# tuanir/fantoch

Hardware: AMD Instinct MI355X
Metric: region configs evaluated/sec (1/2/4/8 GPUs), synthetic 64-region planet n=7 f=1,2 (higher is better)
Workload: dtype u32

## Files before the change

### fantoch_amd/csrc/bote_group.hip

```cpp
#include "bote_fast.hpp"
#include "bote_launch.hpp"

#define AS3 __attribute__((address_space(3)))

namespace bote {

constexpr int GROUP_MAX_BD = 1024;
#ifndef BOTE_GROUP_WAVES
#define BOTE_GROUP_WAVES 5
#endif
#ifndef BOTE_GROUP_WAVES_PERM
#define BOTE_GROUP_WAVES_PERM 4
#endif

__host__ __device__ constexpr int cmax(int a, int b) { return a > b ? a : b; }
template <bool B>
struct BoolC {
  static constexpr bool value = B;
};

template <int N>
struct GCfg {
  using QC = QCfg<N>;
  static constexpr int F = N - 3;
  static constexpr int FP = (F + 1) / 2;
  static constexpr int KQ = cmax(cmax(QC::qa1, QC::maxf >= 2 ? QC::qa2 : 0), cmax(QC::qe, 3)) - 1;
  static_assert(KQ <= N - 1, "quorum larger than the config");
  static constexpr bool PERM = N <= 7 && QC::NL == 2;
  static constexpr bool RX = N <= 7;
  static_assert(!RX || (F <= 4 && KQ <= 4), "position table holds 4 fixed members");
};

__host__ __device__ inline uint32_t gline_rx_bytes(const FastArgs& a, int N) { return N <= 7 && a.grx ? a.ns * 16 : 0u; }
__host__ __device__ inline uint32_t gline_bytes(const FastArgs& a, int N, int KQ) {
  const int F = N - 3, FP = (F + 1) / 2;
  return (gline_rx_bytes(a, N) + a.cq_stride * 8 + (uint32_t)(FP * KQ + 2 * F) * 4 + 15) & ~15u;
}

__host__ __device__ inline uint32_t lines_wave_bytes(const FastArgs& a) {
  return (a.gslots * (a.cq_stride * 8 + 4) + 15) & ~15u;
}

struct GroupLds {
  size_t lines_or_qtab;
  size_t cqt;
  size_t rqt;
  size_t srv;
  size_t lrec;
  size_t cs2;
  size_t vcol;
  size_t vcol32;
  size_t glines;
  size_t top;
  size_t cand;
  size_t tmp;
  size_t thr;
  size_t lock;
  size_t bins;
  size_t digest;
  size_t total;
};

enum : int {
  LOCK_MERGE = 0,
  LOCK_SCORE = 1,
  LOCK_COV = 2,
};

__host__ __device__ inline GroupLds group_layout(const FastArgs& a, int N, int NLW, int KQ, bool perm) {
  const auto a16 = [](size_t o) { return (o + 15) & ~(size_t)15; };
  GroupLds l;
  size_t o = 0;
  l.lines_or_qtab = o; o += perm ? (size_t)(a.gbd / 64) * lines_wave_bytes(a) : ((size_t)N * NLW) << a.gqsh;
  o = a16(o);
  l.cqt = o; o += (size_t)a.R * a.cq_stride * 8;
  l.rqt = o; o += a.rq_separate ? (size_t)a.R * a.rq_stride * 8 : 0;
  l.srv = o; o += (size_t)a.ns * 4;
  o = (o + 7) & ~(size_t)7;
  l.lrec = o; o += (size_t)a.ns * 8;
  o = a16(o);
  l.cs2 = o; o += (size_t)a.ns * 8;
  l.vcol = o; o += (size_t)a.ns * 8;
  l.vcol32 = o; o += (size_t)a.ns * 4;
  o = a16(o);
  l.glines = o; o += (size_t)(a.gbd / 64) * gline_bytes(a, N, KQ);
  o = a16(o);
  l.top = o; o += (size_t)a.n_obj * a.K * 16;
  l.cand = o; o += (size_t)64 * 16;
  l.tmp = o; o += (size_t)a.K * 16;
  l.thr = o; o += (size_t)MAXOBJ * 16;
  l.lock = o; o += 48;
  o = a16(o);
  l.bins = o; o += perm && (a.keys || a.gbins) ? (size_t)(a.gbd / 64) * N * 256 : 0;
  o = a16(o);
  l.digest = o; o += (size_t)a.gbd * 8;
  l.total = o;
  return l;
}

template <int N>
static size_t group_smem_n(const FastArgs& a) {
  return group_layout(a, N, QCfg<N>::NL <= 2 ? 1 : 2, GCfg<N>::KQ, GCfg<N>::PERM).total;
}

bool group_uses_lines(uint32_t n) {
  switch (n) {
#define PL_CASE(NN) case NN: return GCfg<NN>::PERM;
    PL_CASE(4) PL_CASE(5) PL_CASE(6) PL_CASE(7)
#undef PL_CASE
    default: return false;
  }
}

size_t group_smem_bytes(const FastArgs& a, uint32_t n) {
  switch (n) {
#define SM_CASE(NN) case NN: return group_smem_n<NN>(a);
    SM_CASE(4) SM_CASE(5) SM_CASE(6) SM_CASE(7) SM_CASE(8) SM_CASE(9) SM_CASE(10) SM_CASE(11) SM_CASE(12)
    SM_CASE(13) SM_CASE(14) SM_CASE(15) SM_CASE(16)
#undef SM_CASE
    default: return 0;
  }
}

__device__ __forceinline__ uint32_t uni(uint32_t x) { return __builtin_amdgcn_readfirstlane(x); }

__device__ __forceinline__ uint64_t uni64(uint64_t x) {
  return ((uint64_t)uni((uint32_t)(x >> 32)) << 32) | uni((uint32_t)x);
}

__device__ __forceinline__ uint32_t lds_base(const void* p) { return (uint32_t)(uintptr_t)(const AS3 void*)p; }
__device__ __forceinline__ uint32_t l16(uint32_t a) { return *(const AS3 uint16_t*)(uintptr_t)a; }
__device__ __forceinline__ uint32_t l32(uint32_t a) { return *(const AS3 uint32_t*)(uintptr_t)a; }
__device__ __forceinline__ uint2 l64(uint32_t a) {
  const uint64_t v = *(const AS3 uint64_t*)(uintptr_t)a;
  return make_uint2((uint32_t)v, (uint32_t)(v >> 32));
}
typedef uint32_t u32x4 __attribute__((ext_vector_type(4)));
__device__ __forceinline__ uint4 l128(uint32_t a) {
  const u32x4 v = *(const AS3 u32x4*)(uintptr_t)a;
  return make_uint4(v.x, v.y, v.z, v.w);
}
__device__ __forceinline__ float lf32(uint32_t a) { return *(const AS3 float*)(uintptr_t)a; }
__device__ __forceinline__ void s16(uint32_t a, uint32_t v) { *(AS3 uint16_t*)(uintptr_t)a = (uint16_t)v; }
__device__ __forceinline__ void s32(uint32_t a, uint32_t v) { *(AS3 uint32_t*)(uintptr_t)a = v; }
__device__ __forceinline__ void s64(uint32_t a, uint32_t lo, uint32_t hi) {
  *(AS3 uint64_t*)(uintptr_t)a = (uint64_t)lo | ((uint64_t)hi << 32);
}
__device__ __forceinline__ void s128(uint32_t a, uint4 v) {
  u32x4 w;
  w.x = v.x;
  w.y = v.y;
  w.z = v.z;
  w.w = v.w;
  *(AS3 u32x4*)(uintptr_t)a = w;
}

__device__ __forceinline__ void wave_sync() {
  __builtin_amdgcn_fence(__ATOMIC_RELEASE, "workgroup");
  __builtin_amdgcn_wave_barrier();
  __builtin_amdgcn_fence(__ATOMIC_ACQUIRE, "workgroup");
}

__device__ __forceinline__ us2 ld_pair(uint32_t a, uint32_t b) {
  us2 r;
  r.x = *(const AS3 unsigned short*)(uintptr_t)a;
  r.y = *(const AS3 unsigned short*)(uintptr_t)b;
  return r;
}

__device__ __forceinline__ us2 pk_min(us2 a, us2 b) { return __builtin_elementwise_min(a, b); }
__device__ __forceinline__ us2 pk_max(us2 a, us2 b) { return __builtin_elementwise_max(a, b); }

template <int P>
__device__ __forceinline__ void sort_network_pk(uint32_t* a) {
#pragma unroll
  for (int p = 1; p < P; p <<= 1) {
#pragma unroll
    for (int k = p; k >= 1; k >>= 1) {
#pragma unroll
      for (int j = k % p; j + k < P; j += 2 * k) {
#pragma unroll
        for (int i = 0; i < k; ++i) {
          if (i + j + k < P && (i + j) / (2 * p) == (i + j + k) / (2 * p)) {
            const us2 x = as_us2(a[i + j]), y = as_us2(a[i + j + k]);
            a[i + j] = as_u32(pk_min(x, y));
            a[i + j + k] = as_u32(pk_max(x, y));
          }
        }
      }
    }
  }
}

template <int KA, int KY, int KO, class T>
__device__ __forceinline__ void merge_lists(const T* A, const T* y, T* L) {
#pragma unroll
  for (int k = 0; k < KO; ++k) {
    T z = k < KA ? A[k < KA ? k : 0] : y[0];
    bool have = k < KA;
#pragma unroll
    for (int j = 1; j <= KY && j <= k + 1; ++j) {
      const int i = k + 1 - j;
      if (i > KA) continue;
      const T c = i == 0 ? y[j - 1] : __builtin_elementwise_max(A[i > 0 ? i - 1 : 0], y[j - 1]);
      z = have ? __builtin_elementwise_min(z, c) : c;
      have = true;
    }
    L[k] = z;
  }
}

__device__ __forceinline__ int32_t score_tlo(uint64_t tkey, uint32_t nc) {
  if (tkey == ~0ull) return INT32_MIN;
  const uint64_t ob = ~tkey;
  const uint64_t bits = (ob >> 63) ? (ob & 0x7FFFFFFFFFFFFFFFull) : ~ob;
  const double tscore = __longlong_as_double((long long)bits);
  if (!(tscore == tscore)) return INT32_MIN;
  const double b = (tscore - 1e-6) * (double)nc;
  if (b <= -2147483648.0) return INT32_MIN;
  if (b > 1073741824.0) return 1073741824;
  return (int32_t)ceil(b);
}

__device__ __forceinline__ float cov_tf32(uint64_t tkey) {
  if (tkey == ~0ull) return __builtin_inff();
  return (float)__longlong_as_double((long long)tkey) * (1.0f + 0x1p-10f);
}

template <int KA, int KY, class T>
__device__ __forceinline__ void merge_top4(const T* A, const T* y, T* L) {
  static_assert(KA >= 1 && KY >= 1 && KA + KY >= 4 && KA <= 4 && KY <= 4, "4 smallest of KA + KY >= 4 entries");
  T B[4];
#pragma unroll
  for (int i = 0; i < 4; ++i) {
    const int j = 3 - i;
    if (i < KA && j < KY) B[i] = __builtin_elementwise_min(A[i < KA ? i : 0], y[j < KY ? j : 0]);
    else if (i < KA) B[i] = A[i < KA ? i : 0];
    else B[i] = y[j < KY ? j : 0];
  }
  auto ce = [&](int a, int b) {
    const T lo = __builtin_elementwise_min(B[a], B[b]);
    B[b] = __builtin_elementwise_max(B[a], B[b]);
    B[a] = lo;
  };
  ce(0, 2);
  ce(1, 3);
  ce(0, 1);
  ce(2, 3);
#pragma unroll
  for (int i = 0; i < 4; ++i) L[i] = B[i];
}

template <int KA, int KY, int KO, class T>
__device__ __forceinline__ void merge_k(const T* A, const T* y, T* L) {
  if constexpr (KO == 4 && KA + KY >= 4) merge_top4<KA, KY>(A, y, L);
  else merge_lists<KA, KY, KO>(A, y, L);
}

__device__ __forceinline__ void wave_topk(const TopkLds& t, int* lock, uint32_t nc, int n_obj, uint32_t K,
                                          const uint64_t (&key)[MAXOBJ], const bool (&ok)[MAXOBJ], uint64_t rank) {
  const uint32_t lane = threadIdx.x & 63;
  const int KL = (int)K;
  if (lane == 0) {
    while (atomicCAS(lock + LOCK_MERGE, 0, 1) != 0) __builtin_amdgcn_s_sleep(2);
  }
  __builtin_amdgcn_wave_barrier();
  __builtin_amdgcn_fence(__ATOMIC_ACQUIRE, "workgroup");
  const uint32_t rlo = (uint32_t)rank, rhi = (uint32_t)(rank >> 32);
#pragma unroll
  for (int o = 0; o < MAXOBJ; ++o) {
    if (o >= n_obj) break;
    Rec* top = t.top + o * KL;
    const Rec mine = Rec{key[o], rank};
    const bool p = ok[o] && rec_lt(mine, t.thr[o]);
    const uint64_t m = __ballot(p);
    if (m == 0) continue;
    const bool h0 = (int)lane < KL, h1 = (int)lane + 64 < KL;
    const Rec x0 = h0 ? top[lane] : rec_max(), x1 = h1 ? top[lane + 64] : rec_max();
    int r0 = (int)lane, r1 = (int)lane + 64;
    int rc = p ? lower_bound_rec(top, KL, mine) : 0;
    const uint32_t klo = (uint32_t)key[o], khi = (uint32_t)(key[o] >> 32);
    for (uint64_t mm = m; mm; mm &= mm - 1) {
      const int src = __builtin_ctzll(mm);
      const uint64_t ck = ((uint64_t)(uint32_t)__builtin_amdgcn_readlane(khi, src) << 32) |
                          (uint32_t)__builtin_amdgcn_readlane(klo, src);
      const uint64_t cr = ((uint64_t)(uint32_t)__builtin_amdgcn_readlane(rhi, src) << 32) |
                          (uint32_t)__builtin_amdgcn_readlane(rlo, src);
      const Rec c = Rec{ck, cr};
      r0 += rec_lt(c, x0);
      r1 += rec_lt(c, x1);
      rc += rec_lt(c, mine);
    }
    if (h0 && r0 < KL) t.tmp[r0] = x0;
    if (h1 && r1 < KL) t.tmp[r1] = x1;
    if (p && rc < KL) t.tmp[rc] = mine;
    wave_sync();
#pragma unroll
    for (int h = 0; h < KP / 64; ++h)
      if ((int)lane + 64 * h < KL) top[lane + 64 * h] = t.tmp[lane + 64 * h];
    wave_sync();
    if (lane == 0 && rec_lt(top[K - 1], t.thr[o])) {
      t.thr[o] = top[K - 1];
      if (o == 0) lock[LOCK_SCORE] = score_tlo(top[K - 1].key, nc);
      if (o == 3) lock[LOCK_COV] = __float_as_int(cov_tf32(top[K - 1].key));
    }
    wave_sync();
  }
  __builtin_amdgcn_fence(__ATOMIC_RELEASE, "workgroup");
  if (lane == 0) atomicExch(lock + LOCK_MERGE, 0);
}

template <class FX, class FY>
__device__ __forceinline__ int cov2_sign(float Vx, uint32_t Sx, float Vy, uint32_t Sy, const FX& dVx, const FY& dVy) {
  const float fx = (float)Sx, fy = (float)Sy;
  const float x = Vx * (fy * fy), y = Vy * (fx * fx);
  const float d = x - y, tol = 0x1p-18f * fmaxf(x, y);
  if (d < -tol) return -1;
  if (d > tol) return 1;
  const double sx = (double)Sx, sy = (double)Sy;
  const double X = dVx() * (sy * sy), Y = dVy() * (sx * sx);
  const double D = X - Y, T = 0x1p-32 * fmax(X, Y);
  return D < -T ? -1 : (D > T ? 1 : 0);
}

template <class FX, class FY>
__device__ __forceinline__ int cov2_sign_ge(float Vx, uint32_t Sx, float Vy, uint32_t Sy, float fy2, const FX& dVx,
                                            const FY& dVy) {
  const float fx = (float)Sx;
  const float x = Vx * fy2, y = Vy * (fx * fx);
  constexpr float c = 1.0f - 0x1p-18f;
  if (x * c >= y) return 1;
  if (x < y * c) return -1;
  const double sx = (double)Sx, sy = (double)Sy;
  const double X = dVx() * (sy * sy), Y = dVy() * (sx * sx);
  const double D = X - Y, T = 0x1p-32 * fmax(X, Y);
  return D < -T ? -1 : (D > T ? 1 : 0);
}

__device__ __forceinline__ float u64_to_f32(uint64_t x) {
  return __builtin_fmaf((float)(uint32_t)(x >> 32), 0x1p32f, (float)(uint32_t)x);
}

struct GroupCtx {
  bool sid;
  bool use_rx;
  uint32_t LB;
  uint32_t qtab;
  uint32_t cqt, rqt;
  uint32_t thra;
  uint32_t cstride, rstride;
  uint32_t nc, nq, rem;
  uint32_t lines, keys;
  uint32_t rxt;
  uint32_t mfl;
  uint32_t upk;
  uint32_t fS1;
  uint32_t fVf;
};

template <bool LINES>
__device__ __forceinline__ void nearest_quad(const GroupCtx& cx, uint32_t ll, uint32_t c0, uint32_t c1, uint32_t c2,
                                             uint32_t g8, us2& lo, us2& hi) {
  const us2 J1 = {1, 1}, J2 = {2, 2};
  const uint2 wa = l64(c0 + g8);
  if constexpr (LINES) {
    const uint2 wl = l64(ll + g8);
    lo = pk_min(as_us2(wa.x), as_us2(wl.x));
    hi = pk_min(as_us2(wa.y), as_us2(wl.y));
  } else {
    const uint2 wb = l64(c1 + g8), wc = l64(c2 + g8), wf = l64(cx.mfl + g8);
    lo = pk_min(pk_min(as_us2(wa.x), as_us2(wb.x) | J1), pk_min(as_us2(wc.x) | J2, as_us2(wf.x)));
    hi = pk_min(pk_min(as_us2(wa.y), as_us2(wb.y) | J1), pk_min(as_us2(wc.y) | J2, as_us2(wf.y)));
  }
}

template <bool LINES>
__device__ __forceinline__ void nearest_quad_pair(const GroupCtx& cx, uint32_t ll, uint32_t c0, uint32_t c1, uint32_t c2,
                                                  uint32_t g16, us2& lo0, us2& hi0, us2& lo1, us2& hi1) {
  const us2 J1 = {1, 1}, J2 = {2, 2};
  const uint4 wa = l128(c0 + g16);
  if constexpr (LINES) {
    const uint4 wl = l128(ll + g16);
    lo0 = pk_min(as_us2(wa.x), as_us2(wl.x));
    hi0 = pk_min(as_us2(wa.y), as_us2(wl.y));
    lo1 = pk_min(as_us2(wa.z), as_us2(wl.z));
    hi1 = pk_min(as_us2(wa.w), as_us2(wl.w));
  } else {
    const uint4 wb = l128(c1 + g16), wc = l128(c2 + g16), wf = l128(cx.mfl + g16);
    lo0 = pk_min(pk_min(as_us2(wa.x), as_us2(wb.x) | J1), pk_min(as_us2(wc.x) | J2, as_us2(wf.x)));
    hi0 = pk_min(pk_min(as_us2(wa.y), as_us2(wb.y) | J1), pk_min(as_us2(wc.y) | J2, as_us2(wf.y)));
    lo1 = pk_min(pk_min(as_us2(wa.z), as_us2(wb.z) | J1), pk_min(as_us2(wc.z) | J2, as_us2(wf.z)));
    hi1 = pk_min(pk_min(as_us2(wa.w), as_us2(wb.w) | J1), pk_min(as_us2(wc.w) | J2, as_us2(wf.w)));
  }
}

constexpr uint32_t GROUP_UNROLL = 4;
#ifndef BOTE_BIN_FIRST
#define BOTE_BIN_FIRST 0
#endif
#ifndef BOTE_BIN_FIRST_XK
#define BOTE_BIN_FIRST_XK 1
#endif
constexpr uint32_t BIN_UB = 4;
template <int N, bool DEF, bool SI, bool RXC, bool XK, bool BN = false>
__global__ void __launch_bounds__(XK ? GROUP_XK_MAX_BD : GROUP_MAX_BD,
                                  XK ? BOTE_GROUP_WAVES_XK : (GCfg<N>::PERM ? BOTE_GROUP_WAVES_PERM : BOTE_GROUP_WAVES))
    sweep_group_kernel(FastArgs a) {
  GroupCtx cx;
  cx.sid = SI || a.srv_identity;
  constexpr bool S32 = SI;
  cx.use_rx = GCfg<N>::RX && (SI ? RXC : a.grx != 0);
  using QC = QCfg<N>;
  using GC = GCfg<N>;
  constexpr int NL = QC::NL;
  constexpr int NLW = NL <= 2 ? 1 : 2;
  constexpr int F = GC::F;
  constexpr int FP = GC::FP;
  constexpr int KQ = GC::KQ;
  constexpr int PV = Pow2<N - 1>::v;
  constexpr int PF = Pow2<F>::v;
  constexpr bool PERM = GC::PERM;
  constexpr bool BIN = XK || (PERM && BN);
  constexpr bool BIN_FIRST = BIN && (XK ? BOTE_BIN_FIRST_XK : BOTE_BIN_FIRST);
  static_assert(!XK || (PERM && DEF), "the extended key set runs on the PERM kernels with the default objectives");
  using QT = QTab<N, XK>;
  constexpr int NT = QT::NT;
  extern __shared__ __align__(16) unsigned char smem[];
  const GroupLds off = group_layout(a, N, NLW, KQ, PERM);
  cx.LB = lds_base(smem);
  cx.qtab = cx.LB + (uint32_t)off.lines_or_qtab;
  cx.cqt = cx.LB + (uint32_t)off.cqt;
  cx.rqt = cx.LB + (uint32_t)(a.rq_separate ? off.rqt : off.cqt);
  uint32_t* srv = (uint32_t*)(smem + off.srv);
  uint2* lrec = (uint2*)(smem + off.lrec);
  uint64_t* cs2 = (uint64_t*)(smem + off.cs2);
  double* vcol = (double*)(smem + off.vcol);
  float* vcol32 = (float*)(smem + off.vcol32);
  const uint64_t* binom = a.binom;
  TopkLds tk;
  tk.top = (Rec*)(smem + off.top);
  tk.cand = (Rec*)(smem + off.cand);
  tk.tmp = (Rec*)(smem + off.tmp);
  tk.thr = (Rec*)(smem + off.thr);
  cx.thra = cx.LB + (uint32_t)off.thr;
  tk.cnt = nullptr;
  int* lock = (int*)(smem + off.lock);
  const uint32_t tid = threadIdx.x, lane = tid & 63, wid = tid >> 6, BD = blockDim.x, WPB = BD >> 6;
  const uint32_t qsh = a.gqsh;

  {
    const uint32_t cw = a.R * a.cq_stride * 2;
    const uint32_t* src = (const uint32_t*)a.cqt;
    uint32_t* dst = (uint32_t*)(smem + off.cqt);
    for (uint32_t i = tid; i < cw; i += BD) dst[i] = src[i];
    if (a.rq_separate) {
      const uint32_t rw = a.R * a.rq_stride * 2;
      const uint32_t* rs = (const uint32_t*)a.rqt;
      uint32_t* rd = (uint32_t*)(smem + off.rqt);
      for (uint32_t i = tid; i < rw; i += BD) rd[i] = rs[i];
    }
  }
  for (uint32_t i = tid; i < a.ns; i += BD) srv[i] = a.srv[i];
  for (uint32_t i = tid; i < (uint32_t)a.n_obj * a.K; i += BD) tk.top[i] = rec_max();
  if (tid < MAXOBJ) tk.thr[tid] = a.tseed && tid < a.n_obj ? Rec{a.tseed[tid], ~0ull} : rec_max();
  if (tid == 0) {
    lock[LOCK_MERGE] = 0;
    lock[LOCK_SCORE] = score_tlo(a.tseed && a.n_obj ? a.tseed[0] : ~0ull, a.nc);
    lock[LOCK_COV] = __float_as_int(cov_tf32(a.tseed && a.n_obj > 3 ? a.tseed[3] : ~0ull));
  }
  if (a.smin && a.smin_wave && lane < a.n_obj)
    a.smin[(size_t)lane * gridDim.x * WPB + (size_t)blockIdx.x * WPB + wid] = ~0ull;
  if constexpr (BIN)
    for (uint32_t i = tid; i < (BD >> 6) * N * 64; i += BD) ((uint32_t*)(smem + off.bins))[i] = 0;
  ((uint64_t*)(smem + off.digest))[tid] = 0;
  __syncthreads();
  cx.cstride = a.cq_stride * 8;
  cx.rstride = a.rq_stride * 8;
  for (uint32_t i = tid; i < a.ns; i += BD) {
    const uint32_t col = cx.cqt + srv[i] * cx.cstride;
    uint64_t c1 = 0, c2 = 0;
    for (uint32_t c = 0; c < a.nc; ++c) {
      uint64_t v = l16(col + 2 * c) >> LAT_SHIFT;
      c1 += v;
      c2 += v * v;
    }
    cs2[i] = c2;
    const double v = (double)((uint64_t)a.nc * c2 - c1 * c1);
    vcol[i] = v;
    vcol32[i] = (float)v;
    const float w = v > 0.0 ? (float)(1.0 / sqrt(v)) : __builtin_inff();
    lrec[i] = make_uint2((uint32_t)c1, __float_as_uint(w));
  }
  __syncthreads();

  cx.nc = a.nc;
  cx.nq = cx.nc >> 2;
  cx.rem = cx.nc & 3;
  const uint32_t qlane = cx.qtab + tid * 4;
  cx.lines = cx.qtab + wid * lines_wave_bytes(a);
  cx.keys = cx.lines + a.gslots * cx.cstride;
  const uint32_t gl = cx.LB + (uint32_t)off.glines + wid * gline_bytes(a, N, KQ);
  cx.rxt = gl;
  cx.mfl = gl + gline_rx_bytes(a, N);
  cx.upk = cx.mfl + cx.cstride;
  cx.fS1 = cx.upk + FP * KQ * 4;
  cx.fVf = cx.fS1 + F * 4;
  const double pnc1 = a.p_fmean * (double)cx.nc, pnc2 = a.p_emean * (double)cx.nc;
  uint64_t valid_cnt = 0;
  const uint32_t dofs =
      uni(cx.LB + (uint32_t)off.digest + wid * 512u - 2u * (cx.LB + (uint32_t)off.bins + wid * (N * 256u)));
  auto digest_add = [&](uint32_t binb_, uint64_t d) {
    uint32_t ad;
    asm("v_lshl_add_u32 %0, %1, 1, %2" : "=v"(ad) : "v"(binb_), "s"(dofs));
    __hip_atomic_fetch_add((AS3 uint64_t*)(uintptr_t)ad, d, __ATOMIC_RELAXED, __HIP_MEMORY_SCOPE_WAVEFRONT);
  };

  bool static_done = false;
  const uint32_t wsh = a.wshards ? a.wshards : 1u, wx = blockIdx.x % wsh;
  unsigned int* const tctr = a.wctr + 32 * wx;
  uint32_t cnext = 0;
  if (a.nwchunks && lane == 0) cnext = atomicAdd(tctr, 1u);
  for (;;) {
  uint64_t r, rend;
  uint32_t chunk = ~0u;
  if (a.nwchunks) {
    const uint32_t c = wx + wsh * uni(cnext);
    if (c >= a.nwchunks) break;
    if (lane == 0) cnext = atomicAdd(tctr, 1u);
    chunk = c;
    PSTAT(a, 13, true);
    r = uni64(a.wchunks[c]);
    rend = a.smin ? min(r + 64ull * a.ssteps, a.re) : uni64(a.wchunks[c + 1]);
    GASSERT(a, a.rb <= r && r <= rend && rend <= a.re, 0);
  } else {
    if (static_done) break;
    static_done = true;
    const uint64_t nwaves = (uint64_t)gridDim.x * WPB;
    const uint64_t gw = (uint64_t)blockIdx.x * WPB + wid;
    const uint64_t total = a.re - a.rb;
    r = uni64(a.rb + (uint64_t)(((unsigned __int128)total * gw) / nwaves));
    rend = uni64(a.rb + (uint64_t)(((unsigned __int128)total * (gw + 1)) / nwaves));
  }

  if (r < rend) {
    uint32_t hq[F];
    uint64_t base = 0;
    if (a.wstate && chunk != ~0u) {
      const uint64_t* st = a.wstate + 4 * (size_t)chunk;
      base = uni64(st[0]);
      const uint64_t b0 = uni64(st[1]), b1 = uni64(st[2]);
#pragma unroll
      for (int k = 0; k < F; ++k) hq[k] = (uint32_t)((k < 8 ? b0 >> (8 * k) : b1 >> (8 * (k - 8))) & 0xFFu);
    } else {
      uint32_t p[N];
      colex_unrank<N>(binom, a.ns, r, p);
#pragma unroll
      for (int k = 0; k < F; ++k) {
        hq[k] = uni(p[3 + k]);
        base += binom[hq[k] * (N + 1) + (k + 4)];
      }
      base = uni64(base);
    }
    uint64_t low = r - base;
#ifdef BOTE_DEBUG
    {
      bool okq = hq[0] >= 3 && hq[F - 1] < a.ns;
      for (int k = 1; k < F; ++k) okq = okq && hq[k - 1] < hq[k];
      GASSERT(a, okq, 1);
    }
#endif
    for (;;) {
      const uint64_t gend = base + uni64(binom[hq[0] * (N + 1) + 3]);
      PSTAT(a, 12, true);
      uint32_t freg[F];
#pragma unroll
      for (int k = 0; k < F; ++k) freg[k] = uni(cx.sid ? hq[k] : srv[hq[k]]);
      if (lane < (uint32_t)F) {
        uint32_t pos = 0;
#pragma unroll
        for (int k = 0; k < F; ++k) pos = lane == (uint32_t)k ? hq[k] : pos;
        const uint2 lr = lrec[pos];
        s32(cx.fS1 + 4 * lane, lr.x);
        s32(cx.fVf + 4 * lane, lr.y);
      }
      if (lane < (uint32_t)FP) {
        uint32_t v[2][PF];
#pragma unroll
        for (int h = 0; h < 2; ++h) {
          const uint32_t k = 2 * lane + h;
          uint32_t rk = 0;
#pragma unroll
          for (int kk = 0; kk < F; ++kk) rk = k == (uint32_t)kk ? freg[kk] : rk;
#pragma unroll
          for (int m = 0; m < PF; ++m) {
            uint32_t d = 0xFFFFu;
            if (m < F && k < (uint32_t)F && (uint32_t)m != k) d = l16(cx.rqt + freg[m < F ? m : 0] * cx.rstride + 2 * rk) >> LAT_SHIFT;
            v[h][m] = d;
          }
          sort_network<PF>(v[h]);
        }
#pragma unroll
        for (int i = 0; i < KQ; ++i) {
          const uint32_t lo = i < F - 1 ? v[0][i < PF ? i : 0] : 0xFFFFu;
          const uint32_t hi = i < F - 1 ? v[1][i < PF ? i : 0] : 0xFFFFu;
          s32(cx.upk + (lane * KQ + i) * 4, lo | (hi << 16));
        }
      }
      for (uint32_t c = lane; c < (cx.nq + 1) * 4; c += 64) {
        uint32_t key = 3u;
        if (c < cx.nc) {
          key = 0xFFFFu;
#pragma unroll
          for (int k = 0; k < F; ++k) key = min(key, l16(cx.cqt + freg[k] * cx.cstride + 2 * c) | (uint32_t)(3 + k));
        }
        s16(cx.mfl + 2 * c, key);
      }
      GASSERT(a, PERM || (tid + 1) * 4 <= (1u << qsh), 6);
      if (cx.use_rx) {
        GASSERT(a, hq[0] <= a.ns, 5);
        for (uint32_t x = lane; x < hq[0]; x += 64) {
          const uint32_t rg = cx.sid ? x : srv[x];
          uint32_t rf[4], cf[4];
#pragma unroll
          for (int k = 0; k < 4; ++k) {
            const uint32_t fk = freg[k < F ? k : 0];
            rf[k] = k < F ? l16(cx.rqt + fk * cx.rstride + 2 * rg) >> LAT_SHIFT : 0xFFFFu;
            cf[k] = k < F ? l16(cx.rqt + rg * cx.rstride + 2 * fk) >> LAT_SHIFT : 0xFFFFu;
          }
          sort_network<4>(rf);
          s128(cx.rxt + 16 * x, make_uint4(rf[0] | (rf[1] << 16), rf[2] | (rf[3] << 16), cf[0] | (cf[1] << 16),
                                        cf[2] | (cf[3] << 16)));
        }
        if (lane < (uint32_t)F) {
          uint32_t rj = 0, pj = 0;
#pragma unroll
          for (int k = 0; k < F; ++k) {
            rj = lane == (uint32_t)k ? freg[k] : rj;
            pj = lane == (uint32_t)k ? hq[k] : pj;
          }
          uint32_t cf[4];
#pragma unroll
          for (int k = 0; k < 4; ++k) cf[k] = k < F ? l16(cx.rqt + rj * cx.rstride + 2 * freg[k < F ? k : 0]) >> LAT_SHIFT : 0xFFFFu;
          s64(cx.rxt + 16 * pj + 8, cf[0] | (cf[1] << 16), cf[2] | (cf[3] << 16));
        }
      }
      wave_sync();

      const uint64_t cend = uni64(gend < rend ? gend : rend);
      GASSERT(a, low + (cend - r) <= a.lowtab_n, 2);
      uint32_t left = uni((uint32_t)(cend - r)), lo32 = uni((uint32_t)low);
      const uint32_t* ltp = a.lowtab + lo32 + lane;
      uint32_t lp3 = *ltp;
      while (left) {
        const uint32_t len = min(64u, left);
        bool have = lane < len;
        PSTAT(a, 0, true);
        const uint32_t cur = lp3;
        ltp += len;
        if (left > len) lp3 = *ltp;
        uint64_t key[MAXOBJ];
        bool ok[MAXOBJ];
        bool vflag = false;
#pragma unroll
        for (int o = 0; o < MAXOBJ; ++o) {
          key[o] = 0;
          ok[o] = false;
        }
        const uint64_t rank = r + lane;
        uint32_t ll = cx.lines;
        bool use_lines = false;
        if constexpr (PERM) {
          const uint64_t nk = __ballot(have && ((cur & 0xFFu) == 0 || lane == 0));
          const uint32_t nsl = (uint32_t)__popcll(nk);
          use_lines = nsl <= a.gslots && !ABLATE(a, 4096);
          PSTAT(a, 1, !use_lines);
          if (use_lines) {
            const uint32_t below = __builtin_amdgcn_mbcnt_hi((uint32_t)(nk >> 32), __builtin_amdgcn_mbcnt_lo((uint32_t)nk, 0));
            const bool starts = (nk >> lane) & 1;
            const uint32_t slot = below + (starts ? 1u : 0u) - 1;
            ll = cx.lines + slot * cx.cstride;
            GASSERT(a, !have || slot < a.gslots, 4);
            if (starts) s32(cx.keys + 4 * slot, cur);
            wave_sync();
            const uint32_t nqq = cx.nq + (cx.rem ? 1u : 0u);
            const uint32_t lsh = nqq <= 16 ? 3u : (nqq <= 32 ? 4u : 5u), lpl = 1u << lsh;
            const uint32_t li = lane >> lsh, qx = lane & (lpl - 1);
            for (uint32_t sl = 0; sl < nsl; sl += 64u >> lsh) {
              const uint32_t sx = sl + li;
              if (sx < nsl) {
                const uint32_t k = l32(cx.keys + 4 * sx);
                const uint32_t p1 = (k >> 8) & 0xFFu, p2 = k >> 16;
                const uint32_t b1 = cx.cqt + (cx.sid ? p1 : srv[p1]) * cx.cstride;
                const uint32_t b2 = cx.cqt + (cx.sid ? p2 : srv[p2]) * cx.cstride;
                const uint32_t dst = cx.lines + sx * cx.cstride;
                for (uint32_t x = qx; x < nqq; x += lpl) {
                  const uint2 v1 = l64(b1 + 8 * x), v2 = l64(b2 + 8 * x), vf = l64(cx.mfl + 8 * x);
                  const us2 lo = pk_min(pk_min(as_us2(v1.x | 0x00010001u), as_us2(v2.x | 0x00020002u)), as_us2(vf.x));
                  const us2 hi = pk_min(pk_min(as_us2(v1.y | 0x00010001u), as_us2(v2.y | 0x00020002u)), as_us2(vf.y));
                  s64(dst + 8 * x, as_u32(lo), as_u32(hi));
                }
              }
            }
            wave_sync();
          }
        }
        if (have) {
          uint32_t pv[3], rv[3];
          pv[0] = cur & 0xFF;
          pv[1] = (cur >> 8) & 0xFF;
          pv[2] = cur >> 16;
          GASSERT(a, pv[0] < pv[1] && pv[1] < pv[2] && pv[2] < hq[0], 3);
#pragma unroll
          for (int i = 0; i < 3; ++i) rv[i] = cx.sid ? pv[i] : srv[pv[i]];
          uint32_t cv[3];
#pragma unroll
          for (int i = 0; i < 3; ++i) cv[i] = __umul24(rv[i], cx.rstride) + cx.rqt;
          const uint32_t binb = cx.LB + (uint32_t)off.bins + wid * (N * 256) + lane * 4;
          (void)binb;
          auto binned_clients = [&](auto lines_c, uint32_t c0, uint32_t c1, uint32_t c2) -> uint64_t {
            constexpr bool LINES = decltype(lines_c)::value;
            uint32_t s2l = 0;
            uint64_t L2 = 0;
            auto badd = [&](uint32_t addr, uint32_t v) {
              __hip_atomic_fetch_add((AS3 uint32_t*)(uintptr_t)addr, v, __ATOMIC_RELAXED, __HIP_MEMORY_SCOPE_WAVEFRONT);
            };
            auto baddr = [&](uint32_t t) {
              uint32_t r;
              asm("v_lshl_add_u32 %0, %1, 8, %2" : "=v"(r) : "v"(t), "v"(binb));
              return r;
            };
            const uint32_t k256 = 256u;
            auto baddr2 = [&](uint32_t w, uint32_t& lo, uint32_t& hi) {
              const uint32_t t = w & 0x000F000Fu;
              asm("v_mad_u32_u16 %0, %1, %2, %3" : "=v"(lo) : "v"(t), "v"(k256), "v"(binb));
              asm("v_mad_u32_u16 %0, %1, %2, %3 op_sel:[1,0,0,0]" : "=v"(hi) : "v"(t), "v"(k256), "v"(binb));
            };
            const uint32_t kcnt = 0x01000000u, sel_lo = 0x070C0100u, sel_hi = 0x070C0302u;
            auto bval = [&](uint32_t w, uint32_t sel) {
              uint32_t r;
              asm("v_perm_b32 %0, %1, %2, %3" : "=v"(r) : "v"(kcnt), "v"(w), "v"(sel));
              return r;
            };
            auto quad_bin = [&](us2 lo, us2 hi, uint32_t nv) {
              uint32_t L = as_u32(lo), H = as_u32(hi);
#ifdef BOTE_DEBUG
              GASSERT(a, (L & 15u) < (uint32_t)N && ((L >> 16) & 15u) < (uint32_t)N && (H & 15u) < (uint32_t)N &&
                             ((H >> 16) & 15u) < (uint32_t)N, 8);
#endif
              if (nv < 4) {
                L &= nv >= 2 ? ~0u : 0x0000FFFFu;
                H &= nv == 3 ? 0x0000FFFFu : 0u;
              }
              s2l = __builtin_amdgcn_udot2(as_us2(L), as_us2(L), s2l, false);
              s2l = __builtin_amdgcn_udot2(as_us2(H), as_us2(H), s2l, false);
              if (nv >= 4) {
                uint32_t aL0, aL1, aH0, aH1;
                baddr2(L, aL0, aL1);
                baddr2(H, aH0, aH1);
                badd(aL0, bval(L, sel_lo));
                badd(aL1, bval(L, sel_hi));
                badd(aH0, bval(H, sel_lo));
                badd(aH1, bval(H, sel_hi));
                return;
              }
              badd(baddr(L & 15u), __builtin_amdgcn_perm(0x01000000u, L, 0x070C0100u));
              if (nv >= 2) badd(baddr(__builtin_amdgcn_ubfe(L, 16, 4)), __builtin_amdgcn_perm(0x01000000u, L, 0x070C0302u));
              if (nv >= 3) badd(baddr(H & 15u), __builtin_amdgcn_perm(0x01000000u, H, 0x070C0100u));
            };
            constexpr uint32_t UB = LINES ? BIN_UB : 2u;
            const uint32_t nql = ABLATE(a, 1) ? 0u : cx.nq;
            const uint32_t kfl = a.k_flush, fU = kfl / UB ? kfl / UB : 1u;
            uint32_t g = 0, k = 0;
            auto ub_body = [&](uint32_t g0) {
              us2 Lk[UB], Hk[UB];
#pragma unroll
              for (uint32_t u = 0; u < UB; u += 2)
                nearest_quad_pair<LINES>(cx, ll, c0, c1, c2, g0 * 8 + 8 * u, Lk[u], Hk[u], Lk[u + 1], Hk[u + 1]);
#pragma unroll
              for (uint32_t u = 0; u < UB; ++u) quad_bin(Lk[u], Hk[u], 4u);
            };
            if (kfl >= nql + UB) {
              for (; g + 2 * UB <= nql; g += 2 * UB) {
                ub_body(g);
                ub_body(g + UB);
              }
              for (; g + UB <= nql; g += UB) ub_body(g);
            } else if (kfl >= UB) {
              for (; g + UB <= nql; g += UB) {
                us2 Lk[UB], Hk[UB];
#pragma unroll
                for (uint32_t u = 0; u < UB; u += 2)
                  nearest_quad_pair<LINES>(cx, ll, c0, c1, c2, g * 8 + 8 * u, Lk[u], Hk[u], Lk[u + 1], Hk[u + 1]);
#pragma unroll
                for (uint32_t u = 0; u < UB; ++u) quad_bin(Lk[u], Hk[u], 4u);
                if (++k == fU) {
                  L2 += s2l;
                  s2l = 0;
                  k = 0;
                }
              }
              L2 += s2l;
              s2l = 0;
            }
            for (; g < nql; ++g) {
              us2 Lk, Hk;
              nearest_quad<LINES>(cx, ll, c0, c1, c2, g * 8, Lk, Hk);
              quad_bin(Lk, Hk, 4u);
              L2 += s2l;
              s2l = 0;
            }
            if (cx.rem && !ABLATE(a, 1)) {
              us2 Lk, Hk;
              nearest_quad<LINES>(cx, ll, c0, c1, c2, cx.nq * 8, Lk, Hk);
              quad_bin(Lk, Hk, cx.rem);
            }
            return L2 + s2l;
          };
          uint64_t L2first = 0;
          if constexpr (BIN && BIN_FIRST) {
            const uint32_t f0 = __umul24(rv[0], cx.cstride) + cx.cqt, f1 = __umul24(rv[1], cx.cstride) + cx.cqt,
                           f2 = __umul24(rv[2], cx.cstride) + cx.cqt;
            L2first = use_lines ? binned_clients(BoolC<true>{}, f0, f1, f2) : binned_clients(BoolC<false>{}, f0, f1, f2);
          }
          uint32_t Q2[N], Q3[N];
          uint32_t Q2w[4] = {0u, 0u, 0u, 0u}, Q3w[4] = {0u, 0u, 0u, 0u};
          uint32_t cS1p = 0, cS1e = 0;
          uint32_t cS2[NT], cS1t[NT];
#pragma unroll
          for (int t = 0; t < NT; ++t) cS2[t] = cS1t[t] = 0;
          uint32_t wp[NT][2 + FP];
          auto emit_pk = [&](int j, bool has_hi, const uint32_t* L) {
            const uint32_t w0 = L[QC::lq(0) - 2], w1 = L[(NL >= 2 ? QC::lq(1) : QC::lq(0)) - 2];
            if constexpr (PERM) {
              Q2[j] = L[0] & 0xFFFFu;
              Q3[j] = L[1] & 0xFFFFu;
              if (has_hi) {
                Q2[j + 1] = L[0] >> 16;
                Q3[j + 1] = L[1] >> 16;
              }
              const int pi = j == 0 ? 0 : (j == 2 ? 1 : 2 + (j - 3) / 2);
              const uint32_t hm = has_hi ? ~0u : 0xFFFFu;
#pragma unroll
              for (int t = 0; t < NT; ++t) wp[t][pi] = L[QT::q(t) - 2] & hm;
              Q2w[pi] = L[0] & hm;
              Q3w[pi] = L[1] & hm;
              (void)w0;
              (void)w1;
              return;
            }
#pragma unroll
            for (int h = 0; h < 2; ++h) {
              if (h == 1 && !has_hi) break;
              const uint32_t sel = h ? 0x07060302u : 0x05040100u;
              const uint32_t sh = h ? 16u : 0u;
              Q2[j + h] = (L[0] >> sh) & 0xFFFFu;
              Q3[j + h] = (L[1] >> sh) & 0xFFFFu;
              const uint32_t word = NL >= 2 ? __builtin_amdgcn_perm(w1, w0, sel) : ((w0 >> sh) & 0xFFFFu);
              if (!ABLATE(a, 1024)) s32(qlane + ((uint32_t)(j + h) << qsh), word);
              cS1p += word;
              const uint32_t q0 = word & 0xFFFFu;
              cS2[0] += q0 * q0;
              if (NL >= 2) {
                const uint32_t q1 = word >> 16;
                cS2[NL >= 2 ? 1 : 0] += q1 * q1;
              }
              if (NL == 3) {
                const uint32_t q2 = (L[QC::lq(NL - 1) - 2] >> sh) & 0xFFFFu;
                s32(qlane + ((uint32_t)(N + j + h) << qsh), q2);
                cS1e += q2;
                cS2[NL - 1] += q2 * q2;
              }
            }
          };
          if (cx.use_rx) {
            uint4 X0, X1, X2;
            if (ABLATE(a, 8192)) {
              X0 = make_uint4(pv[0], pv[1], pv[2], pv[0] ^ pv[1]);
              X1 = make_uint4(pv[2], pv[0], pv[1], pv[1] ^ pv[2]);
              X2 = make_uint4(pv[1], pv[2], pv[0], pv[0] ^ pv[2]);
            } else {
              X0 = l128(cx.rxt + 16 * pv[0]);
              X1 = l128(cx.rxt + 16 * pv[1]);
              X2 = l128(cx.rxt + 16 * pv[2]);
            }
            {
              us2 A[4], y[2], L[KQ];
              A[0] = as_us2(__builtin_amdgcn_perm(X1.x, X0.x, 0x05040100u));
              A[1] = as_us2(__builtin_amdgcn_perm(X1.x, X0.x, 0x07060302u));
              A[2] = as_us2(__builtin_amdgcn_perm(X1.y, X0.y, 0x05040100u));
              A[3] = as_us2(__builtin_amdgcn_perm(X1.y, X0.y, 0x07060302u));
              y[0] = as_us2((l16(cv[1] + 2 * rv[0]) | (l16(cv[0] + 2 * rv[1]) << 16)) >> LAT_SHIFT);
              y[1] = as_us2((l16(cv[2] + 2 * rv[0]) | (l16(cv[2] + 2 * rv[1]) << 16)) >> LAT_SHIFT);
              const us2 t = pk_min(y[0], y[1]);
              y[1] = pk_max(y[0], y[1]);
              y[0] = t;
              if (ABLATE(a, 32)) {
#pragma unroll
                for (int k = 0; k < KQ; ++k) L[k] = pk_min(A[k], y[k & 1]);
              } else {
                merge_k<F < 4 ? F : 4, 2, KQ>(A, y, L);
              }
              uint32_t W[KQ];
#pragma unroll
              for (int k = 0; k < KQ; ++k) W[k] = as_u32(L[k]);
              emit_pk(0, true, W);
            }
            {
              uint32_t A[4], y[2], L[KQ];
              A[0] = X2.x & 0xFFFFu;
              A[1] = X2.x >> 16;
              A[2] = X2.y & 0xFFFFu;
              A[3] = X2.y >> 16;
              const uint32_t d20 = l16(cv[0] + 2 * rv[2]) >> LAT_SHIFT, d21 = l16(cv[1] + 2 * rv[2]) >> LAT_SHIFT;
              y[0] = min(d20, d21);
              y[1] = max(d20, d21);
              merge_k<F < 4 ? F : 4, 2, KQ>(A, y, L);
              emit_pk(2, false, L);
            }
#pragma unroll
            for (int pp = 0; pp < FP; ++pp) {
              us2 A[KQ];
#pragma unroll
              for (int i = 0; i < KQ; ++i) A[i] = as_us2(l32(cx.upk + (pp * KQ + i) * 4));
              const bool has_hi = 2 * pp + 1 < F;
              us2 y[3];
              y[0] = as_us2(pp == 0 ? X0.z : X0.w);
              y[1] = as_us2(pp == 0 ? X1.z : X1.w);
              y[2] = as_us2(pp == 0 ? X2.z : X2.w);
              {
                us2 t = pk_min(y[0], y[1]);
                y[1] = pk_max(y[0], y[1]);
                y[0] = t;
                t = pk_min(y[1], y[2]);
                y[2] = pk_max(y[1], y[2]);
                y[1] = t;
                t = pk_min(y[0], y[1]);
                y[1] = pk_max(y[0], y[1]);
                y[0] = t;
              }
              us2 L[KQ];
              if (ABLATE(a, 64)) {
#pragma unroll
                for (int k = 0; k < KQ; ++k) L[k] = pk_min(A[k], y[k < 3 ? k : 2]);
              } else {
                merge_k<(F - 1 < KQ ? F - 1 : KQ), 3, KQ>(A, y, L);
              }
              uint32_t W[KQ];
#pragma unroll
              for (int k = 0; k < KQ; ++k) W[k] = as_u32(L[k]);
              emit_pk(3 + 2 * pp, has_hi, W);
            }
          } else {
            {
              uint32_t v[PV];
              v[0] = (l16(cv[1] + 2 * rv[0]) | (l16(cv[0] + 2 * rv[1]) << 16)) >> LAT_SHIFT;
              v[1] = (l16(cv[2] + 2 * rv[0]) | (l16(cv[2] + 2 * rv[1]) << 16)) >> LAT_SHIFT;
  #pragma unroll
              for (int k = 0; k < F; ++k) {
                const uint32_t fc = cx.rqt + freg[k] * cx.rstride;
                v[2 + k] = (l16(fc + 2 * rv[0]) | (l16(fc + 2 * rv[1]) << 16)) >> LAT_SHIFT;
              }
  #pragma unroll
              for (int k = N - 1; k < PV; ++k) v[k] = 0xFFFFFFFFu;
              if (!ABLATE(a, 32)) sort_network_pk<PV>(v);
              emit_pk(0, true, v);
            }
            {
              uint32_t v[PV];
              v[0] = l16(cv[0] + 2 * rv[2]) >> LAT_SHIFT;
              v[1] = l16(cv[1] + 2 * rv[2]) >> LAT_SHIFT;
  #pragma unroll
              for (int k = 0; k < F; ++k) v[2 + k] = l16(cx.rqt + freg[k] * cx.rstride + 2 * rv[2]) >> LAT_SHIFT;
  #pragma unroll
              for (int k = N - 1; k < PV; ++k) v[k] = 0xFFFFu;
              if (!ABLATE(a, 32)) sort_network<PV>(v);
              emit_pk(2, false, v);
            }
  #pragma unroll
            for (int pp = 0; pp < FP; ++pp) {
              us2 A[KQ];
  #pragma unroll
              for (int i = 0; i < KQ; ++i) A[i] = as_us2(l32(cx.upk + (pp * KQ + i) * 4));
              const bool has_hi = 2 * pp + 1 < F;
              us2 y[3];
  #pragma unroll
              for (int m = 0; m < 3; ++m) {
                const uint32_t lo = l16(cv[m] + 2 * freg[2 * pp]);
                const uint32_t hi = has_hi ? l16(cv[m] + 2 * freg[has_hi ? 2 * pp + 1 : 2 * pp]) : 0xFFF0u;
                y[m] = as_us2((lo | (hi << 16)) >> LAT_SHIFT);
                if (!has_hi) y[m] = as_us2(as_u32(y[m]) | 0xFFFF0000u);
              }
              {
                us2 t = pk_min(y[0], y[1]);
                y[1] = pk_max(y[0], y[1]);
                y[0] = t;
                t = pk_min(y[1], y[2]);
                y[2] = pk_max(y[1], y[2]);
                y[1] = t;
                t = pk_min(y[0], y[1]);
                y[1] = pk_max(y[0], y[1]);
                y[0] = t;
              }
              uint32_t L[KQ];
  #pragma unroll
              for (int k = 0; k < KQ; ++k) {
                us2 z = A[k];
// ... 700 lines not shown
```

Baseline: 49.34 billion.

## Reuse last line slot across chunks and flatten line-building loop with 128-bit LDS ops

Line building in the permutation path now keeps a ring of slots, so when a new 64-rank chunk starts with the same (p1,p2) key as the previous chunk's last line, that line is reused instead of rebuilt. The per-slot nested loop becomes a single flattened loop over (slot, 16-byte piece), using a magic-multiply divide and 128-bit LDS loads and stores. Key entries now hold precomputed row base addresses (8 bytes per slot), which removes the srv lookups and multiplies from the inner loop. This aims to cut redundant LDS work and improve lane utilisation, at the cost of slightly more LDS per wave and ring-index bookkeeping.

```diff
diff --git a/fantoch_amd/csrc/bote_group.hip b/fantoch_amd/csrc/bote_group.hip
--- a/fantoch_amd/csrc/bote_group.hip
+++ b/fantoch_amd/csrc/bote_group.hip
@@ -38,7 +38,7 @@
 }
 
 __host__ __device__ inline uint32_t lines_wave_bytes(const FastArgs& a) {
-  return (a.gslots * (a.cq_stride * 8 + 4) + 15) & ~15u;
+  return (a.gslots * (a.cq_stride * 8 + 8) + 15) & ~15u;
 }
 
 struct GroupLds {
@@ -351,6 +351,7 @@
   uint32_t cstride, rstride;
   uint32_t nc, nq, rem;
   uint32_t lines, keys;
+  uint32_t npieces, pmagic;
   uint32_t rxt;
   uint32_t mfl;
   uint32_t upk;
@@ -499,6 +500,8 @@
   const uint32_t qlane = cx.qtab + tid * 4;
   cx.lines = cx.qtab + wid * lines_wave_bytes(a);
   cx.keys = cx.lines + a.gslots * cx.cstride;
+  cx.npieces = uni((cx.nq + (cx.rem ? 1u : 0u) + 1) >> 1);
+  cx.pmagic = uni(65536u / (cx.npieces ? cx.npieces : 1u) + 1);
   const uint32_t gl = cx.LB + (uint32_t)off.glines + wid * gline_bytes(a, N, KQ);
   cx.rxt = gl;
   cx.mfl = gl + gline_rx_bytes(a, N);
@@ -651,6 +654,7 @@
       uint32_t left = uni((uint32_t)(cend - r)), lo32 = uni((uint32_t)low);
       const uint32_t* ltp = a.lowtab + lo32 + lane;
       uint32_t lp3 = *ltp;
+      uint32_t lkey = ~0u, lslot = 0;
       while (left) {
         const uint32_t len = min(64u, left);
         bool have = lane < len;
@@ -675,33 +679,41 @@
           use_lines = nsl <= a.gslots && !ABLATE(a, 4096);
           PSTAT(a, 1, !use_lines);
           if (use_lines) {
+            const uint32_t reuse = (uni(cur) >> 8) == lkey ? 1u : 0u;
+            const uint32_t sbase = reuse ? lslot : 0u;
+            auto ring = [&](uint32_t s) { return min(s, s - a.gslots); };
             const uint32_t below = __builtin_amdgcn_mbcnt_hi((uint32_t)(nk >> 32), __builtin_amdgcn_mbcnt_lo((uint32_t)nk, 0));
             const bool starts = (nk >> lane) & 1;
-            const uint32_t slot = below + (starts ? 1u : 0u) - 1;
+            const uint32_t slot = ring(sbase + below + (starts ? 1u : 0u) - 1);
             ll = cx.lines + slot * cx.cstride;
             GASSERT(a, !have || slot < a.gslots, 4);
-            if (starts) s32(cx.keys + 4 * slot, cur);
+            if (starts) {
+              const uint32_t p1 = (cur >> 8) & 0xFFu, p2 = cur >> 16;
+              s64(cx.keys + 8 * slot, cx.cqt + __umul24(cx.sid ? p1 : srv[p1], cx.cstride),
+                  cx.cqt + __umul24(cx.sid ? p2 : srv[p2], cx.cstride));
+            }
             wave_sync();
-            const uint32_t nqq = cx.nq + (cx.rem ? 1u : 0u);
-            const uint32_t lsh = nqq <= 16 ? 3u : (nqq <= 32 ? 4u : 5u), lpl = 1u << lsh;
-            const uint32_t li = lane >> lsh, qx = lane & (lpl - 1);
-            for (uint32_t sl = 0; sl < nsl; sl += 64u >> lsh) {
-              const uint32_t sx = sl + li;
-              if (sx < nsl) {
-                const uint32_t k = l32(cx.keys + 4 * sx);
-                const uint32_t p1 = (k >> 8) & 0xFFu, p2 = k >> 16;
-                const uint32_t b1 = cx.cqt + (cx.sid ? p1 : srv[p1]) * cx.cstride;
-                const uint32_t b2 = cx.cqt + (cx.sid ? p2 : srv[p2]) * cx.cstride;
-                const uint32_t dst = cx.lines + sx * cx.cstride;
-                for (uint32_t x = qx; x < nqq; x += lpl) {
-                  const uint2 v1 = l64(b1 + 8 * x), v2 = l64(b2 + 8 * x), vf = l64(cx.mfl + 8 * x);
-                  const us2 lo = pk_min(pk_min(as_us2(v1.x | 0x00010001u), as_us2(v2.x | 0x00020002u)), as_us2(vf.x));
-                  const us2 hi = pk_min(pk_min(as_us2(v1.y | 0x00010001u), as_us2(v2.y | 0x00020002u)), as_us2(vf.y));
-                  s64(dst + 8 * x, as_u32(lo), as_u32(hi));
-                }
-              }
+            const uint32_t nit = (nsl - reuse) * cx.npieces;
+            PSTAT(a, 14, reuse != 0);
+            for (uint32_t i = lane; i < nit; i += 64) {
+              PSTAT(a, 15, true);
+              const uint32_t j = __umul24(i, cx.pmagic) >> 16, g16 = (i - j * cx.npieces) * 16;
+              const uint32_t sx = ring(sbase + reuse + j);
+              const uint2 b = l64(cx.keys + 8 * sx);
+              const uint4 v1 = l128(b.x + g16), v2 = l128(b.y + g16), vf = l128(cx.mfl + g16);
+              uint4 o;
+              o.x = as_u32(pk_min(pk_min(as_us2(v1.x | 0x00010001u), as_us2(v2.x | 0x00020002u)), as_us2(vf.x)));
+              o.y = as_u32(pk_min(pk_min(as_us2(v1.y | 0x00010001u), as_us2(v2.y | 0x00020002u)), as_us2(vf.y)));
+              o.z = as_u32(pk_min(pk_min(as_us2(v1.z | 0x00010001u), as_us2(v2.z | 0x00020002u)), as_us2(vf.z)));
+              o.w = as_u32(pk_min(pk_min(as_us2(v1.w | 0x00010001u), as_us2(v2.w | 0x00020002u)), as_us2(vf.w)));
+              s128(cx.lines + __umul24(sx, cx.cstride) + g16, o);
             }
             wave_sync();
+            lkey = uni(__builtin_amdgcn_readlane(cur, len - 1)) >> 8;
+            lslot = sbase + nsl - 1;
+            lslot = lslot >= a.gslots ? lslot - a.gslots : lslot;
+          } else {
+            lkey = ~0u;
           }
         }
         if (have) {
```

Result: no change. 49.16 billion (-0.4%).
